# tingliu/glia

Measured on AMD Instinct MI355X. Metric: region_merges_per_sec, higher is better.
Workload: dtype u32 labels / f32 image / f64 statistics and features

## Files before the change

### glia_amd/csrc/api.cpp

```cpp
#include <algorithm>
#include <atomic>
#include <chrono>
#include <cmath>
#include <cstdio>
#include <cstdlib>
#include <cstring>
#include <limits>
#include <mutex>
#include <unordered_map>

#include "bc_features.hpp"
#include "forest.hpp"
#include "rmap_order.hpp"
#include "hmt_internal.hpp"

namespace glia {

static thread_local std::string g_err;
void set_error(const std::string& msg) { g_err = msg; }

static const char* const kOptionKeys[] = {"GLIA_HMT_PB_WINDOW", "GLIA_HMT_PB_BATCH", "GLIA_HMT_WINCAP", "GLIA_HMT_REBASE", "GLIA_HMT_HORIZON",
                                          "GLIA_HMT_FORCE_TREE", "GLIA_HMT_HELPERS", "GLIA_HMT_TRACE", "GLIA_HMT_LIBM", "GLIA_HMT_BC_NOCOMMON",
                                          "GLIA_HMT_BC_GENERIC", "GLIA_HMT_DEBUG", "GLIA_HMT_MAXITERS", "GLIA_HMT_MINCAP"};
static std::mutex g_opt_mu;
// ... 717 lines not shown
  }
  if (type != 1 && type != 2 && type != 3) {
    set_error("Error: unsupported boundary stats type...");
    return GLIA_HMT_ERR_ARG;
  }
  GLIA_HIP_TRY(hipSetDevice(c->device));
  *n_merges = 0;
  if (rag->arr.R == 0 || rag->arr.P == 0) return GLIA_HMT_OK;
  PbRequest req;
  if (type == 1 || type == 3) req.median_of = &rag->vol;
  req.size_weight = type == 3;
  MergeResult res;
  const int rc = greedy_mean(rag->arr, c->stream, req, &res);
  if (rc) return rc;
  rag->ms_table = res.ms_table; rag->ms_loop = res.ms_loop; rag->n_scored = res.n_scored;
  return order_to_keys(rag, res, "merge_order_pb", rag->only_contour, capacity, h_order, h_sal, n_merges);
}

static int upload_forest(const HostForest& hf, glia_hmt_forest* f, int slot, hipStream_t stream) {
  std::vector<PackedNode> nodes;
  std::vector<int> roots;
  int rc = pack_forest(hf, &nodes, &roots);
  if (rc) return rc;
  PackedNode* d_nodes = nullptr;
  int* d_roots = nullptr;
  GLIA_HIP_TRY(hipMalloc(&d_nodes, sizeof(PackedNode) * nodes.size()));
  f->allocs.push_back(d_nodes);
  GLIA_HIP_TRY(hipMalloc(&d_roots, sizeof(int) * roots.size()));
  f->allocs.push_back(d_roots);
  GLIA_HIP_TRY(hipMemcpyAsync(d_nodes, nodes.data(), sizeof(PackedNode) * nodes.size(), hipMemcpyHostToDevice, stream));
// ... 156 lines not shown
    set_error("pre_merge: invalid argument");
    return GLIA_HMT_ERR_ARG;
  }
  if (rag->only_contour) { set_error("pre_merge: the region map must hold region points (only_contour = 0)"); return GLIA_HMT_ERR_ARG; }
  GLIA_HIP_TRY(hipSetDevice(c->device));
  *n_merges = 0;
  if (rag->arr.R == 0 || rag->arr.P == 0) return GLIA_HMT_OK;
  PbRequest req;
  req.cond_n = n_thresholds;
  req.cond_sizes[0] = size_thresholds[0]; req.cond_sizes[1] = n_thresholds > 1 ? size_thresholds[1] : 0;
  req.cond_rpb = rpb_threshold;
  MergeResult res;
  const int rc = greedy_mean(rag->arr, c->stream, req, &res);
  if (rc) return rc;
  rag->ms_table = res.ms_table; rag->ms_loop = res.ms_loop; rag->n_scored = res.n_scored;
  return order_to_keys(rag, res, "pre_merge", false, capacity, h_order, h_sal, n_merges);
}

int glia_hmt_bc_feat(glia_hmt_ctx* c, glia_hmt_rag* rag, const uint32_t* h_order, int64_t n_merges, double* h_feats) {
  return glia_hmt_bc_feat_saliency(c, rag, h_order, n_merges, nullptr, 1.0, 1.0, h_feats);
}

int glia_hmt_bc_feat_dim(const glia_hmt_rag* rag, int with_saliency) {
  BcCfg cfg;
  if (!rag || !make_bc_cfg(rag, &cfg)) return -1;
  return cfg.fdim + median_extra_cols(rag, cfg) + ((with_saliency && !cfg.use_simple) ? 5 : 0);
}

int glia_hmt_bc_feat_saliency(glia_hmt_ctx* c, glia_hmt_rag* rag, const uint32_t* h_order, int64_t n_merges,
                              const double* h_saliencies, double init_saliency, double saliency_bias, double* h_feats) {
// ... 298 lines not shown
  if (!r || !out) return GLIA_HMT_ERR_ARG;
  *out = r->bcl;
  return GLIA_HMT_OK;
}

int glia_hmt_last_merge_timing(const glia_hmt_rag* r, double* ms_table, double* ms_init, double* ms_loop,
                               int64_t* n_scored) {
  if (!r) return GLIA_HMT_ERR_ARG;
  if (ms_table) *ms_table = r->ms_table;
  if (ms_init) *ms_init = r->ms_init;
  if (ms_loop) *ms_loop = r->ms_loop;
  if (n_scored) *n_scored = r->n_scored;
  return GLIA_HMT_OK;
}

}
```

### glia_amd/csrc/api_types.hpp

```cpp
#pragma once
#include "glibc_math.hpp"
#include "greedy_common.hpp"
#include "hmt_internal.hpp"

using namespace glia;

struct glia_hmt_ctx {
  int device = 0;
  hipStream_t stream = nullptr;
  bool own_stream = false;
  uint32_t rcap = 0, pcap = 0;
  uint32_t* rkeys = nullptr; uint32_t* rrec = nullptr;
  unsigned long long* pkeys = nullptr; uint32_t* prec = nullptr;
  uint32_t* flags = nullptr;
  hipEvent_t ev0 = nullptr, ev1 = nullptr;
  uint32_t hint_rcap = 0, hint_pcap = 0;
  double transform_ms = 0;
  int tz = kTZ;
  LibmSel libm = {kLibmDevice, kLibmDevice, kLibmDevice};
};

struct glia_hmt_rag {
  glia_hmt_ctx* ctx = nullptr;
  int dim = 3;
  int64_t dims[3] = {1, 1, 1};
  bool only_contour = false;
  int bins = 0, nthr = 0;
  RagArrays arr;
  double pass_ms = 0, alg_bytes = 0;
  double ms_table = 0, ms_init = 0, ms_loop = 0;
  glia_hmt_bc_label_timing bcl;
  int64_t n_scored = 0;
  glia_hmt_feat_config cfg;
  bool has_cfg = false;
  VolumeRef vol;
  VolumeRef slab;
  uint32_t* d_folded = nullptr;
  int map_region[GLIA_HMT_MAX_IMAGES] = {0}, map_rlabel[GLIA_HMT_MAX_IMAGES] = {0}, map_boundary[GLIA_HMT_MAX_IMAGES] = {0};
};
```

### glia_amd/csrc/greedy.hip

```cpp
#include <atomic>
#include <cstring>
#include <vector>
#include <limits>
#include <rocprim/device/device_scan.hpp>
#include <rocprim/device/device_radix_sort.hpp>
#include <rocprim/device/device_segmented_radix_sort.hpp>

#include "greedy_batch.hpp"

namespace glia {

__global__ void pq_build_level_kernel(PqTree t, int l) {
  const int lane = threadIdx.x & 63;
  uint32_t j = (blockIdx.x * blockDim.x + threadIdx.x) >> 6;
  if (j < t.lv[l].size) (void)pq_recompute_node(t, l, j, lane, true);
}

int pq_setup(DeviceBuffers& buf, PqTree& t, hipStream_t stream) {
  t.nlevels = 0;
  uint32_t n = t.nleaves;
  while (true) {
    n = (n + kFan - 1) / kFan;
    if (t.nlevels >= kMaxLevels) { set_error("greedy: edge table too large"); return GLIA_HMT_ERR_ARG; }
    PqLevel& L = t.lv[t.nlevels++];
// ... 22 lines not shown
namespace {

__global__ void win_range_kernel(const double* sal, uint32_t E0, unsigned long long* mm) {
  unsigned long long lo = ~0ull, hi = 0ull;
  for (uint32_t i = blockIdx.x * blockDim.x + threadIdx.x; i < E0; i += gridDim.x * blockDim.x) {
    const unsigned long long b = f64_ord(sal[i]);
    lo = b < lo ? b : lo; hi = b > hi ? b : hi;
  }
  atomicMin(&mm[0], lo); atomicMax(&mm[1], hi);
}
__global__ void win_params_kernel(const unsigned long long* mm, uint32_t B, double* range) {
  const double smin = f64_unord(mm[0]), smax = f64_unord(mm[1]);
  range[0] = smin;
  range[1] = smax > smin ? (double)B / (smax - smin) : 0.0;
}
__global__ void win_collect_kernel(const EdgeRec* er, uint32_t n_edges, const uint8_t* rdead, unsigned long long* kseq, uint32_t* vals, uint32_t* counter) {
  const uint32_t e = blockIdx.x * blockDim.x + threadIdx.x;
  if (e >= n_edges) return;
  const unsigned long long q = er[e].seq;
  if (q == 0) return;
  const uint2 uv = *reinterpret_cast<const uint2*>(&er[e].u);
  if (rdead[uv.x] | rdead[uv.y]) return;
  const uint32_t i = atomicAdd(counter, 1u);
  kseq[i] = q; vals[i] = e;
}
__global__ void win_salkey_kernel(const EdgeRec* er, const uint32_t* vals, uint32_t n, unsigned long long* ksal) {
  const uint32_t i = blockIdx.x * blockDim.x + threadIdx.x;
  if (i < n) ksal[i] = f64_ord(er[vals[i]].sal);
}
__global__ void win_baseline_fill_kernel(WinState st, uint32_t n, uint32_t* isort_w, unsigned long long* isort_seq) {
  const uint32_t i = blockIdx.x * blockDim.x + threadIdx.x;
  if (i >= n) return;
  const EdgeRec r = st.er[isort_w[i]];
  isort_seq[i] = r.seq;
  atomicAdd(&st.wcnt[win_cell(r.sal, st.wrange[0], st.wrange[1], st.wB)], 1u);
}
__global__ void win_segments_kernel(WinState st, const uint32_t* isort, uint32_t n, uint32_t* ige) {
  const uint32_t c = blockIdx.x * blockDim.x + threadIdx.x;
  if (c > st.wB) return;
// ... 128 lines not shown
  st.e_mean[e] = med;
  st.pq.leaf_sal[e] = st.size_weight ? -med * (double)min(st.rsz[st.e_u[e]], st.rsz[st.e_v[e]]) : -med;
  atomicAdd(&st.rbv[st.e_u[e]], (unsigned long long)n);
  atomicAdd(&st.rbv[st.e_v[e]], (unsigned long long)n);
}

__global__ void fill_leaves_dead(PqTree t, uint32_t from) {
  uint32_t i = from + blockIdx.x * blockDim.x + threadIdx.x;
  if (i < t.nleaves) { t.leaf_seq[i] = 0; t.leaf_sal[i] = -__builtin_inf(); }
}

}

struct WinBaseline {
  unsigned long long *kseq = nullptr, *kseq2 = nullptr, *ksal = nullptr, *ksal2 = nullptr, *iseq = nullptr;
  uint32_t *vals = nullptr, *vals2 = nullptr, *isort = nullptr, *ige = nullptr, *counter = nullptr;
  void* tmp = nullptr; size_t tmp_bytes = 0;
  uint32_t E0 = 0;
  double h_range[2] = {0.0, 0.0};
  long long prev_top_cell = -1;
  unsigned long long prev_ne = 0;
  double horizon_factor = 0.0;

  int init(DeviceBuffers& buf, WinState& ws, const double* leaf_sal, uint32_t n_initial, uint32_t B, uint32_t R, hipStream_t stream) {
    int rc;
    E0 = n_initial;
    unsigned long long* mm; double* range;
    if ((rc = buf.get(&ws.rdead, 2 * (size_t)R, true, stream))) return rc;
    if ((rc = buf.get(&ws.whead, B, false, stream))) return rc;
    if ((rc = buf.get(&ws.wcnt, B, true, stream))) return rc;
    if ((rc = buf.get(&isort, E0, false, stream))) return rc;
    if ((rc = buf.get(&iseq, E0, false, stream))) return rc;
    if ((rc = buf.get(&ige, (size_t)B + 1, false, stream))) return rc;
    if ((rc = buf.get(&mm, 2, false, stream))) return rc;
    if ((rc = buf.get(&range, 2, false, stream))) return rc;
    if ((rc = buf.get(&kseq, E0, false, stream))) return rc;
    if ((rc = buf.get(&kseq2, E0, false, stream))) return rc;
    if ((rc = buf.get(&ksal, E0, false, stream))) return rc;
    if ((rc = buf.get(&ksal2, E0, false, stream))) return rc;
    if ((rc = buf.get(&vals, E0, false, stream))) return rc;
    if ((rc = buf.get(&vals2, E0, false, stream))) return rc;
    if ((rc = buf.get(&counter, 1, true, stream))) return rc;
    GLIA_HIP_TRY(rocprim::radix_sort_pairs_desc(nullptr, tmp_bytes, kseq, kseq2, vals, vals2, (size_t)E0, 0, 64, stream));
    if ((rc = buf.get((char**)&tmp, tmp_bytes ? tmp_bytes : 16, false, stream))) return rc;
    ws.wrange = range; ws.isort = isort; ws.isort_seq = iseq; ws.ige = ige;
    const unsigned long long mm0[2] = {~0ull, 0ull};
    GLIA_HIP_TRY(hipMemcpyAsync(mm, mm0, sizeof(mm0), hipMemcpyHostToDevice, stream));
    hipLaunchKernelGGL(win_range_kernel, dim3(256), dim3(256), 0, stream, leaf_sal, E0, mm);
    hipLaunchKernelGGL(win_params_kernel, dim3(1), dim3(1), 0, stream, mm, B, range);
    GLIA_HIP_TRY(hipGetLastError());
    GLIA_HIP_TRY(hipMemcpyAsync(h_range, range, sizeof(h_range), hipMemcpyDeviceToHost, stream));
    GLIA_HIP_TRY(hipStreamSynchronize(stream));
    return GLIA_HMT_OK;
  }
  int rebaseline(WinState& ws, uint32_t n_edges, unsigned long long* ctrl, hipStream_t stream) {
    GLIA_HIP_TRY(hipMemsetAsync(counter, 0, sizeof(uint32_t), stream));
    hipLaunchKernelGGL(win_collect_kernel, dim3((n_edges + 255) / 256), dim3(256), 0, stream, ws.er, n_edges, ws.rdead, kseq, vals, counter);
    uint32_t n = 0;
    GLIA_HIP_TRY(hipMemcpyAsync(&n, counter, sizeof(uint32_t), hipMemcpyDeviceToHost, stream));
    GLIA_HIP_TRY(hipStreamSynchronize(stream));
    if (n > E0) { set_error("greedy: more live edges than initial edges (internal error)"); return GLIA_HMT_ERR_INTERNAL; }
    if (n) {
      size_t bytes = tmp_bytes;
      GLIA_HIP_TRY(rocprim::radix_sort_pairs_desc(tmp, bytes, kseq, kseq2, vals, vals2, (size_t)n, 0, 64, stream));
      hipLaunchKernelGGL(win_salkey_kernel, dim3((n + 255) / 256), dim3(256), 0, stream, ws.er, vals2, n, ksal);
      bytes = tmp_bytes;
      GLIA_HIP_TRY(rocprim::radix_sort_pairs_desc(tmp, bytes, ksal, ksal2, vals2, isort, (size_t)n, 0, 64, stream));
    }
    GLIA_HIP_TRY(hipMemsetAsync(ws.whead, 0xFF, sizeof(uint32_t) * ws.wB, stream));
    GLIA_HIP_TRY(hipMemsetAsync(ws.wcnt, 0, sizeof(uint32_t) * ws.wB, stream));
    if (n) hipLaunchKernelGGL(win_baseline_fill_kernel, dim3((n + 255) / 256), dim3(256), 0, stream, ws, n, isort, iseq);
    hipLaunchKernelGGL(win_segments_kernel, dim3((ws.wB + 1 + 255) / 256), dim3(256), 0, stream, ws, isort, n, ige);
    GLIA_HIP_TRY(hipGetLastError());
    ws.nsort = n;
    std::string renv;
    ws.rebase_after = option("GLIA_HMT_REBASE", &renv) ? strtoull(renv.c_str(), nullptr, 10) : std::max<unsigned long long>(800000ull, (unsigned long long)n / 2ull);
    ws.wch = 0;
    if (horizon_factor > 0.0 && n > 4096) {
      unsigned long long topkey = 0;
      GLIA_HIP_TRY(hipMemcpyAsync(&topkey, ksal2, sizeof(topkey), hipMemcpyDeviceToHost, stream));
      GLIA_HIP_TRY(hipStreamSynchronize(stream));
      const long long top_cell = (long long)win_cell(f64_unord(topkey), h_range[0], h_range[1], ws.wB);
      if (prev_top_cell >= 0 && n_edges > prev_ne) {
        const double d = (double)std::max<long long>(0, prev_top_cell - top_cell);
        const double delta = std::max(horizon_factor * d * (double)ws.rebase_after / (double)(n_edges - prev_ne), (double)ws.wB / 512.0);
        ws.wch = (double)top_cell > delta ? (uint32_t)((double)top_cell - delta) : 0u;
      }
      prev_top_cell = top_cell; prev_ne = n_edges;
    }
    ws.ne_base = n_edges;
    const double inf = std::numeric_limits<double>::infinity();
    ctrl[CTRL_CTHR] = (unsigned long long)(long long)(ws.wB - 1);
    memcpy(&ctrl[CTRL_TSAL], &inf, 8); ctrl[CTRL_TSEQ] = ~0ull; ctrl[CTRL_IPTR] = 0;
    return GLIA_HMT_OK;
  }
};
// ... 103 lines not shown
    ws.wB = B; ws.R0 = R;
    ws.wcap = kWinCap; ws.wbudget = kWinBudget;
    ws.force_tree = 0;
    if (option("GLIA_HMT_FORCE_TREE", &o_txt)) ws.force_tree = strtoull(o_txt.c_str(), nullptr, 10);
    if (option("GLIA_HMT_WINCAP", &o_txt)) {
      const uint32_t c = (uint32_t)strtoul(o_txt.c_str(), nullptr, 10);
      if (c >= 16 && c <= kWinCap) { ws.wcap = c; ws.wbudget = c / 2; }
    }
    ws.order = st.order; ws.sal_out = st.sal_out; ws.ctrl = st.ctrl; ws.rsz = st.rsz; ws.rsum = st.rsum;
    ws.mark0 = st.mark0; ws.mark1 = st.mark1; ws.adj_off = st.adj_off; ws.adj_len = st.adj_len;
    ws.pool_cap = st.pool_cap; ws.Ecap = st.Ecap;
    ws.cond_n = st.cond_n; ws.cond_t0 = st.cond_t0; ws.cond_t1 = st.cond_t1; ws.cond_rpb = st.cond_rpb;
    if ((rc = base.init(buf, ws, st.pq.leaf_sal, E0, B, R, stream))) return rc;
    if (req.cond_n <= 0 && !batch_off) base.horizon_factor = option("GLIA_HMT_HORIZON", &o_txt) ? atof(o_txt.c_str()) : 0.5;
    if ((rc = base.rebaseline(ws, E0, ctrl, stream))) return rc;
  } else if ((rc = pq_setup(buf, st.pq, stream))) return rc;
  GLIA_HIP_TRY(hipMemcpyAsync(st.ctrl, ctrl, sizeof(ctrl), hipMemcpyHostToDevice, stream));
  GLIA_HIP_TRY(hipEventRecord(ev.ev[1], stream));


  st.max_iters = window ? 1ull << 22 : 1ull << 16;
  const bool trace = option("GLIA_HMT_TRACE");
  if (option("GLIA_HMT_MAXITERS", &o_txt)) st.max_iters = std::max(1ull, strtoull(o_txt.c_str(), nullptr, 10));
  const auto kernel = [&]() { return !window ? "tree" : req.cond_n > 0 ? "window" : "batch"; };
  const auto unhandled = [&]() {
    set_error(std::string("greedy: the ") + kernel() + " kernel stopped with status " + std::to_string(ctrl[CTRL_STATUS]) + ", which its driver does not handle (internal error)");
    return GLIA_HMT_ERR_INTERNAL;
  };
  while (true) {
    if (window) {
      ws.max_iters = st.max_iters;
      if (req.cond_n > 0) hipLaunchKernelGGL(greedy_window_kernel<true>, dim3(1), dim3(kGreedyThreads), 0, stream, ws);
      else if (batch_off) hipLaunchKernelGGL(greedy_window_kernel<false>, dim3(1), dim3(kGreedyThreads), 0, stream, ws);
      else hipLaunchKernelGGL(greedy_batch_kernel, dim3(1), dim3(kGreedyThreads), 0, stream, ws);
    } else if (median_of) hipLaunchKernelGGL(greedy_pb_kernel<true>, dim3(1), dim3(kGreedyThreads), 0, stream, st);
    else hipLaunchKernelGGL(greedy_pb_kernel<false>, dim3(1), dim3(kGreedyThreads), 0, stream, st);
    GLIA_HIP_TRY(hipGetLastError());
    GLIA_HIP_TRY(hipMemcpyAsync(ctrl, st.ctrl, sizeof(ctrl), hipMemcpyDeviceToHost, stream));
    GLIA_HIP_TRY(hipStreamSynchronize(stream));
    if (trace) fprintf(stderr, "[trace] merge loop launch ended: status %llu, merges %llu of %u regions, edges %llu, list entries %llu\n", ctrl[CTRL_STATUS], ctrl[CTRL_MERGES], R, ctrl[CTRL_EDGES], ctrl[CTRL_ENTRIES]);
    if (ctrl[CTRL_STATUS] == ST_DONE) break;
    switch (ctrl[CTRL_STATUS]) {
      case ST_RUN:
        if (!window) continue;
        break;
      case ST_REBASE:
        if (!window) return unhandled();
        break;
      case ST_BAD_SALIENCY: set_error("Error: invalid boundary saliency..."); return GLIA_HMT_ERR_SALIENCY;
      case ST_INTERNAL: {
        char msg[256];
        snprintf(msg, sizeof(msg), "greedy: window queue overflow or more merges than regions (internal error: merges %llu of %u regions, %llu edges of %u initial, "
// ... 27 lines not shown
        break;
      }
      case ST_NEED_EDGES: {
        if (st.Ecap >= kMaxEdgeSlots) { set_error("greedy: more than 2^32 edge slots needed"); return GLIA_HMT_ERR_ARG; }
        const uint32_t ocap = st.Ecap, ncap = (uint32_t)std::min<unsigned long long>(kMaxEdgeSlots, (unsigned long long)ocap * 2ull);
        if ((rc = edges.grow(buf, ocap, ncap, stream))) return rc;
        st.Ecap = ncap; st.pq.nleaves = ncap; ws.Ecap = ncap;
        hipLaunchKernelGGL(fill_leaves_dead, dim3((ncap - ocap + 255) / 256), dim3(256), 0, stream, st.pq, ocap);
        if (!window && (rc = pq_setup(buf, st.pq, stream))) return rc;
        break;
      }
      default: return unhandled();
    }
    if (window) {
      if ((rc = base.rebaseline(ws, (uint32_t)ctrl[CTRL_EDGES], ctrl, stream))) return rc;
      GLIA_HIP_TRY(hipMemcpyAsync(st.ctrl + CTRL_CTHR, ctrl + CTRL_CTHR, 4 * sizeof(unsigned long long), hipMemcpyHostToDevice, stream));
    }
    unsigned long long zero = ST_RUN;
    GLIA_HIP_TRY(hipMemcpyAsync(st.ctrl + CTRL_STATUS, &zero, sizeof(zero), hipMemcpyHostToDevice, stream));
  }
  GLIA_HIP_TRY(hipEventRecord(ev.ev[2], stream));
  GLIA_HIP_TRY(hipEventSynchronize(ev.ev[2]));
  out->ms_table = ev.ms(0, 1); out->ms_loop = ev.ms(1, 2);
  out->n_scored = (int64_t)ctrl[CTRL_EDGES];
  return copy_merges(out, (int64_t)ctrl[CTRL_MERGES], st.order, st.sal_out);
}


static std::atomic<unsigned long long> g_internal_errors{0};
unsigned long long internal_errors() { return g_internal_errors.load(); }
void count_internal_error() { g_internal_errors.fetch_add(1); }
bool merge_order_is_consistent(const uint32_t* o, int64_t n, uint32_t R, int64_t* first_bad) {
  std::vector<uint8_t> gone(2 * (size_t)R + 1, 0);
  for (int64_t k = 0; k < n; ++k) {
    const uint32_t a = o[3 * k], b = o[3 * k + 1], c = o[3 * k + 2];
    if (k >= (int64_t)R || c != R + (uint32_t)k || a >= c || b >= c || a == b || gone[a] || gone[b]) { if (first_bad) *first_bad = k; return false; }
    gone[a] = gone[b] = 1;
  }
  return true;
// ... 17 lines not shown
```

### glia_amd/csrc/greedy_batch.hpp

```cpp
#pragma once
#include "greedy_window.hpp"

namespace glia {
namespace {

constexpr uint32_t kBatchKill = 32;
constexpr int kMemP = 3;
constexpr uint32_t kMemMax = 192;
struct BatchShared {
  alignas(16) Key part1[kNW];
  alignas(16) Key part2[kNW];
  uint32_t nkill, kovf; alignas(16) uint32_t kill[kBatchKill];
  uint32_t byrank[kNW];
  uint32_t bitmap[kNW][64];
  uint32_t m_newcount[kNW], m_total[kNW], m_ok[kNW];
  double m_maxsal[kNW];
  uint32_t bad;
};

template <int CTRL, int ROW_MASK = 0xf>
__device__ __forceinline__ void top2_ord_step(unsigned long long& a1, unsigned long long& a2) {
  const unsigned long long b1 = dpp64<CTRL, ROW_MASK, ROW_MASK != 0xf>(a1), b2 = dpp64<CTRL, ROW_MASK, ROW_MASK != 0xf>(a2);
  const bool g = b1 > a1;
  const unsigned long long hi = g ? b1 : a1, lo = g ? a1 : b1, m2 = b2 > a2 ? b2 : a2;
  a1 = hi; a2 = lo > m2 ? lo : m2;
}
__device__ __forceinline__ void wave_top2_ord(unsigned long long& a1, unsigned long long& a2) {
  top2_ord_step<0xB1>(a1, a2);
  top2_ord_step<0x4E>(a1, a2);
  top2_ord_step<0x124>(a1, a2);
  top2_ord_step<0x128>(a1, a2);
  top2_ord_step<0x142, 0xa>(a1, a2);
// ... 188 lines not shown
  lds_barrier();
  WIDE_T(5);
  if (tid == 0) { s.nitems = 0; s.newcount = 0; }
  *newcount_out = newcount;
  return total;
}

__global__ __launch_bounds__(kGreedyThreads) void greedy_batch_kernel(WinState st) {
  __shared__ WinShared w;
  __shared__ WinWork s;
  __shared__ BatchShared b;
  const int tid = threadIdx.x, lane = tid & 63, wave = tid >> 6;
  unsigned long long k = st.ctrl[CTRL_MERGES], ne = st.ctrl[CTRL_EDGES], pool_used = st.ctrl[CTRL_ENTRIES];
  uint32_t status = ST_RUN;
  win_enter(st, w, s, tid);
  if (tid == 0) { b.nkill = 0; b.kovf = 0; b.bad = 0; }
  b.bitmap[wave][lane] = 0;
  if (tid < kNW) { Key z; z.sal = -__builtin_inf(); z.seq = 0; z.arg = 0; b.part1[tid] = z; b.part2[tid] = z; }
  full_barrier();
  const double smin = st.wrange[0], scale = st.wrange[1];
  uint32_t pend_e = kNone, pend_old = kNone;
  constexpr uint32_t kTab = kMarkSlots / kNW;
  uint32_t* const tk = &s.mk[wave * kTab]; uint32_t* const t0 = &s.mv0[wave * kTab]; uint32_t* const t1 = &s.mv1[wave * kTab];
  static_assert(sizeof(s.stage) >= (size_t)kNW * kTab * 20, "per-wave staging");
  uint32_t* const sg_eid = reinterpret_cast<uint32_t*>(&s.stage[0]) + wave * kTab;
  uint32_t* const sg_n = reinterpret_cast<uint32_t*>(&s.stage[0]) + (kNW + wave) * kTab;
  uint32_t* const sg_pos = reinterpret_cast<uint32_t*>(&s.stage[0]) + (2 * kNW + wave) * kTab;
  double* const sg_mean = reinterpret_cast<double*>(reinterpret_cast<uint32_t*>(&s.stage[0]) + 3 * kNW * kTab) + wave * kTab;
#ifdef GLIA_HMT_PROFILE
  unsigned long long bph[8] = {0, 0, 0, 0, 0, 0, 0, 0}, blast = __builtin_readcyclecounter(), brounds = 0, bmembers = 0, bvalid = 0, bwide = 0, bcut_sal = 0, bcut_dep = 0;
  unsigned long long bw_n[4] = {0, 0, 0, 0}, bw_cyc[4] = {0, 0, 0, 0}, bw_ent[4] = {0, 0, 0, 0}, bw_new[4] = {0, 0, 0, 0};
// ... 46 lines not shown
    if (top_total > kMemMax) {
      if (ne + top_total > st.Ecap) { status = ST_NEED_EDGES; break; }
      if (pool_used + top_total > st.pool_cap) { status = ST_NEED_POOL; break; }
      uint32_t newcount = 0;
#ifdef GLIA_HMT_PROFILE
      const unsigned long long tw0 = __builtin_readcyclecounter();
#endif
      const uint32_t tt = batch_contract_wide(st, w, s, b, tid, top.arg, top.sal, k, ne, pool_used, smin, scale, &newcount);
      if (b.bad) { status = ST_BAD_SALIENCY; break; }
      k += 1; ne += newcount; pool_used += tt;
#ifdef GLIA_HMT_PROFILE
      bwide += 1;
      { const int cls = tt <= 512u ? 0 : tt <= kMarkMax ? 1 : tt <= 8192u ? 2 : 3; bw_n[cls] += 1; bw_cyc[cls] += __builtin_readcyclecounter() - tw0; bw_ent[cls] += tt; bw_new[cls] += newcount; }
#endif
      batch_scan(st, w, b, tid, kScanWide);
      if (w.spill_ord) { if (pend_e != kNone) { st.er[pend_e].next = pend_old; pend_e = kNone; } win_evict(st, w, tid); batch_scan(st, w, b, tid, kScanOther); }
      BPH(4);
      continue;
    }
    const bool narrow = member && total <= kMemMax;
    b.bitmap[wave][lane] = 0;
    FatEntry fe[kMemP];
    bool act[kMemP], side1[kMemP];
    uint32_t h[kMemP];
#pragma unroll
    for (int p = 0; p < kMemP; ++p) {
      const uint32_t i = (uint32_t)lane + 64u * (uint32_t)p;
      const bool inlist = narrow && i < total;
      side1[p] = i >= len0;
      fe[p].eid = kNone; fe[p].rs = 0; fe[p].n = 0; fe[p].pos = 0; fe[p].off = 0; fe[p].len = 0; fe[p].mean = 0.0;
      if (inlist) fe[p] = st.fpool[side1[p] ? off1 + (i - len0) : off0 + i];
// ... 73 lines not shown
      V = (uint32_t)__builtin_ctz(~okbits);
#ifdef GLIA_HMT_PROFILE
      if (V < M) { const uint32_t cutsal = (uint32_t)(__ballot(lane < kNW && j == V && !(kj.sal > pm)) & 0xFFull); if (cutsal) bcut_sal += 1; else bcut_dep += 1; }
#endif
      my_ne = (uint32_t)__builtin_amdgcn_readlane((int)pre_n, wave); my_pool = (uint32_t)__builtin_amdgcn_readlane((int)pre_t, wave);
      const uint32_t last = V - 1u;
      ne_off = (uint32_t)__shfl((int)(pre_n + nj), (int)last); pool_off = (uint32_t)__shfl((int)(pre_t + tj), (int)last);
    }
    const uint32_t sum_tot = pool_off;
    if (ne + sum_tot > st.Ecap) { status = ST_NEED_EDGES; break; }
    if (pool_used + sum_tot > st.pool_cap) { status = ST_NEED_POOL; break; }
    bool popped = false;
    if (wn_round + ne_off > st.wcap && wn_round > st.wcap / 2u) {
      if ((uint32_t)wave < V && lane == 0) w.seq[slot] = 0;
      popped = true;
      lds_barrier();
      win_compact(w, tid, st.wcap);
    }
    const WinTau tau = {w.cthr, w.tsal, w.tseq, smin, scale};
    BPH(2);
    if ((uint32_t)wave < V) {
      const unsigned long long kk = k + (unsigned long long)wave;
      const uint32_t r2 = st.R0 + (uint32_t)kk;
      const uint32_t r2off = (uint32_t)pool_used + my_pool;
      if (lane == 0) {
        if (!popped) w.seq[slot] = 0;
        st.order[3 * kk + 0] = r0; st.order[3 * kk + 1] = r1; st.order[3 * kk + 2] = r2;
        st.sal_out[kk] = me.sal;
        st.er[e].seq = 0;
        st.rdead[r0] = 1; st.rdead[r1] = 1;
// ... 10 lines not shown
        const unsigned long long seq = update_seq(kk, rs, r0, h0);
        const double sal = -first[p];
        store_new_edge(st, newE, rs, r2, posRs, idx[p], first[p], second[p], sal, seq, offRs, lenRs, r2off, newcount);
        win_queue_edge<true>(st, w, tau, newE, sal, seq, rs, r2, make_uint2(offRs, lenRs), make_uint2(r2off, newcount), pend_e, pend_old);
        win_retire_edge<true, false, kBatchKill>(st, tau, fe[p].eid, -fe[p].mean, &b.nkill, b.kill, &b.kovf);
        if (both[p]) win_retire_edge<true, false, kBatchKill>(st, tau, p_eid[p], -p_mean[p], &b.nkill, b.kill, &b.kovf);
      }
    }
    lds_barrier();
    BPH(3);
#ifdef GLIA_HMT_PROFILE
    brounds += 1; bmembers += M; bvalid += V;
#endif
    k += V; ne += ne_off; pool_used += pool_off;
    batch_scan(st, w, b, tid, kScanNarrow);
    if (w.spill_ord) { if (pend_e != kNone) { st.er[pend_e].next = pend_old; pend_e = kNone; } win_evict(st, w, tid); batch_scan(st, w, b, tid, kScanOther); }
    BPH(4);
  }
#ifdef GLIA_HMT_PROFILE
  if (tid == 0) printf("[batch profile] merges %llu: select %llu  compute %llu  validate %llu  commit %llu  scan %llu  loop-top %llu  reload %llu (cycles); rounds %llu candidates %llu committed %llu (cut by saliency %llu, by adjacency %llu) wide %llu\n",
                       k, bph[0], bph[1], bph[2], bph[3], bph[4], bph[5], bph[6], brounds, bmembers, bvalid, bcut_sal, bcut_dep, bwide);
  if (tid == 0) printf("[batch profile] scan phases (cumulative cycles, wave 0): loads %llu  compare %llu  top2 %llu  top2 with a tied best %llu  barrier %llu  calls %llu  tied second %llu  tied best %llu\n",
                       g_scanprof[0], g_scanprof[1], g_scanprof[2], g_scanprof[3], g_scanprof[4], g_scanprof[7], g_scanprof[5], g_scanprof[6]);
  if (tid == 0) printf("[batch profile] scan fill (cumulative; n <= 512, <= 1024, more): after reload/evict %llu %llu %llu  after narrow round %llu %llu %llu  after wide %llu %llu %llu\n",
                       g_scanfill[0][0], g_scanfill[0][1], g_scanfill[0][2], g_scanfill[1][0], g_scanfill[1][1], g_scanfill[1][2], g_scanfill[2][0], g_scanfill[2][1], g_scanfill[2][2]);
  if (tid == 0) printf("[batch profile] loop top (this launch): narrow rounds %llu cycles %llu  wide pops %llu cycles %llu\n", bsel_n[0], bsel[0], bsel_n[1], bsel[1]);
  if (tid == 0) printf("[batch profile] wide phases (cumulative cycles): entry-barrier %llu  lists+table %llu  compact %llu  main loop (wave 0) %llu  loop barrier %llu  tail %llu\n",
                       g_wideprof[0], g_wideprof[1], g_wideprof[2], g_wideprof[3], g_wideprof[4], g_wideprof[5]);
  if (tid == 0) printf("[batch profile] wide by entries (<=512, <=1408, <=8192, more): n %llu %llu %llu %llu  cycles %llu %llu %llu %llu  entries %llu %llu %llu %llu  new edges %llu %llu %llu %llu\n",
                       bw_n[0], bw_n[1], bw_n[2], bw_n[3], bw_cyc[0], bw_cyc[1], bw_cyc[2], bw_cyc[3], bw_ent[0], bw_ent[1], bw_ent[2], bw_ent[3], bw_new[0], bw_new[1], bw_new[2], bw_new[3]);
#endif
  if (pend_e != kNone) st.er[pend_e].next = pend_old;
  full_barrier();
  win_leave(st, w, tid, k, ne, pool_used, status);
}

}
}
```

### glia_amd/csrc/greedy_tree.hpp

```cpp
#pragma once
#include "greedy_common.hpp"

namespace glia {

struct GreedyState {
  uint32_t R0;
  uint32_t* adj_off;
  uint32_t* adj_len;
  uint2* pool;
  unsigned long long pool_cap;
  uint32_t Ecap;
  uint32_t *e_u, *e_v, *e_posu, *e_posv;
  double* e_mean;
  int* e_n;
  float* vals;
  unsigned long long vals_cap;
  unsigned long long* e_off;
  unsigned long long* rbv;
  int size_weight;
  PqTree pq;
  int cond_n; unsigned long long cond_t0, cond_t1; double cond_rpb;
  unsigned long long* rsz;
  double* rsum;
  uint32_t *mark0, *mark1;
  uint32_t* order;
  double* sal_out;
  unsigned long long* ctrl;
  unsigned long long max_iters;
};
enum { CTRL_MERGES = 0, CTRL_EDGES = 1, CTRL_ENTRIES = 2,
       CTRL_STATUS = 3, CTRL_VALUES = 4,
       CTRL_CTHR = 5, CTRL_TSAL = 6, CTRL_TSEQ = 7, CTRL_IPTR = 8,
       CTRL_WERR = 9, CTRL_WFILL = 10, CTRL_WORDS = 11 };

namespace {

__device__ __forceinline__ bool mean_link(bool h0, double m0, int n0, bool h1, double m1, int n1, double* first, int* second) {
  double f = 0.0;
  int sc = 0;
  if (h0) { f += m0 * n0; sc += n0; }
  if (h1) { f += m1 * n1; sc += n1; }
  f = sdivide(f, (double)sc, 0.0);
  *first = f; *second = sc;
  return f == -1.0;
}
__device__ __forceinline__ unsigned long long update_seq(unsigned long long k, uint32_t rs, uint32_t r0, bool h0) {
  const uint32_t cat = rs < r0 ? 0u : (h0 ? 1u : 2u);
  return ((k + 1ull) << 32) | ((unsigned long long)cat << 30) | rs;
// ... 358 lines not shown
```

### glia_amd/csrc/hmt_internal.hpp

```cpp
#pragma once
#include <hip/hip_runtime.h>
#include <stdint.h>
#include <string>
#include <vector>

#include "../../include/glia_hmt.h"

namespace glia {

void set_error(const std::string& msg);
bool option(const char* key, std::string* value = nullptr);
unsigned long long internal_errors();
void count_internal_error();
bool merge_order_is_consistent(const uint32_t* dense_order, int64_t n, uint32_t R, int64_t* first_bad);
int finish_merge_order(int rc, const uint32_t* dense_order, int64_t n, uint32_t R, hipStream_t stream);
#define GLIA_HIP_TRY(expr)                                                                       \
  do {                                                                                           \
    hipError_t _e = (expr);                                                                      \
    if (_e != hipSuccess) {                                                                      \
      ::glia::set_error(std::string(#expr) + ": " + hipGetErrorString(_e));                      \
      return GLIA_HMT_ERR_HIP;                                                                   \
    }                                                                                            \
  } while (0)

// ... 82 lines not shown
};
int median_feature_stats(const MedianFeatIn& in, hipStream_t stream, std::vector<double>* reg, std::vector<double>* bnd, std::vector<unsigned long long>* area);
struct TruthCount { uint32_t leaf, truth; unsigned long long count; };
int truth_overlap(const VolumeRef& vol, const uint32_t* d_rlabel, uint32_t R, const uint32_t* d_truth, hipStream_t stream,
                  std::vector<TruthCount>* out, float* ms);
struct NodeTruthStats { std::vector<unsigned long long> n, size, Q; std::vector<long double> E; };
void node_truth_stats(const std::vector<TruthCount>& cnt, uint32_t R, const uint32_t* forced, int64_t M, NodeTruthStats* out, int64_t* moves,
                      int64_t* node_pairs);
int bc_label_rules(const std::vector<NodeTruthStats>& st, uint32_t R, const uint32_t* forced, int64_t M, const glia_hmt_bc_label_opts& o,
                   int32_t* labels);
struct MergeResult {
  std::vector<uint32_t> order;
  std::vector<double> sal, rows;
  int64_t n = 0, n_scored = 0;
  double ms_table = 0.0, ms_init = 0.0, ms_loop = 0.0;
};
struct PbRequest {
  int cond_n = 0;
  long long cond_sizes[2] = {0, 0};
  double cond_rpb = 0.0;
  const VolumeRef* median_of = nullptr;
  bool size_weight = false;
};
int greedy_mean(const RagArrays& rag, hipStream_t stream, const PbRequest& req, MergeResult* out);
struct BcCfg;
struct DeviceClassifier;
struct BcRequest {
  const uint32_t* forced = nullptr;
  int64_t n_forced = 0;
  bool rows = false;
// ... 43 lines not shown
```

### glia_amd/hmt.py

```python
import ctypes as C
import os

import numpy as np

_HERE = os.path.dirname(os.path.abspath(__file__))
_SO = os.environ.get("GLIA_HMT_LIB", os.path.join(_HERE, "libglia_hmt.so"))

MAX_IMAGES, MAX_BINS, MAX_THRESH = 8, 16, 4


class HmtError(RuntimeError):
    def __init__(self, code, msg):
        super().__init__("glia_hmt error %d: %s" % (code, msg))
        self.code = code


class Image(C.Structure):
    _fields_ = [("d_image", C.c_void_p), ("bins", C.c_int), ("lo", C.c_double), ("hi", C.c_double)]


class FeatConfig(C.Structure):
    _fields_ = [
        ("n_region", C.c_int), ("region", Image * MAX_IMAGES),
        ("n_rlabel", C.c_int), ("rlabel", Image * MAX_IMAGES),
# ... 611 lines not shown

    def boundary_confidence(self, trees):
        import torch
        nt = len(trees)
        keep = [[np.ascontiguousarray(t[0], np.uint32), np.ascontiguousarray(t[1], np.int32), np.ascontiguousarray(t[2], np.int32),
                 np.ascontiguousarray(t[4], np.float64)] for t in trees]
        nn = (C.c_int64 * nt)(*[len(k[0]) for k in keep])
        arr = lambda j: (C.c_void_p * nt)(*[k[j].ctypes.data for k in keep])
        out = torch.empty(self.shape, dtype=torch.float32, device=torch.device("cuda", self.ctx.device))
        _check(lib().glia_hmt_boundary_confidence(self.ctx.h, self.h, C.c_int(nt), nn, arr(0), arr(1), arr(2), arr(3), C.c_void_p(out.data_ptr())))
        return out

    def last_merge_timing(self):
        a, b, c, n = C.c_double(), C.c_double(), C.c_double(), C.c_int64()
        _check(lib().glia_hmt_last_merge_timing(self.h, C.byref(a), C.byref(b), C.byref(c), C.byref(n)))
        return dict(ms_table=a.value, ms_init=b.value, ms_loop=c.value, n_edges_scored=n.value)
```

### include/glia_hmt.h

```cpp
#ifndef GLIA_HMT_H
#define GLIA_HMT_H

#include <stdint.h>

#ifdef __cplusplus
extern "C" {
#endif

#define GLIA_HMT_OK 0
#define GLIA_HMT_ERR_ARG (-1)
#define GLIA_HMT_ERR_HIP (-2)
#define GLIA_HMT_ERR_UNSUPPORTED (-3)
#define GLIA_HMT_ERR_CAPACITY (-4)
#define GLIA_HMT_ERR_SALIENCY (-5)
#define GLIA_HMT_ERR_IO (-6)
#define GLIA_HMT_ERR_INTERNAL (-7)

#define GLIA_HMT_MAX_IMAGES 8
#define GLIA_HMT_MAX_BINS 16
#define GLIA_HMT_MAX_THRESH 4

typedef struct glia_hmt_ctx glia_hmt_ctx;
typedef struct glia_hmt_rag glia_hmt_rag;
typedef struct glia_hmt_forest glia_hmt_forest;
// ... 162 lines not shown

int glia_hmt_relabel_image(glia_hmt_ctx* ctx, uint32_t* d_labels, int64_t n_voxels, int64_t min_size, uint32_t* n_labels);

double glia_hmt_last_transform_ms(const glia_hmt_ctx* ctx);

int64_t glia_hmt_gen_tree(const uint32_t* h_order, int64_t n_merges, uint32_t* node_label, int32_t* parent,
                          int32_t* child0, int32_t* child1, int64_t capacity);

int glia_hmt_score_initial_edges(glia_hmt_ctx* ctx, glia_hmt_rag* rag, const glia_hmt_forest* forest,
                                 int64_t* n_edges, double* ms);
int glia_hmt_score_initial_edges_shard(glia_hmt_ctx* ctx, glia_hmt_rag* rag, const glia_hmt_forest* forest, int shard,
                                       int n_shards, double* h_scores, int64_t capacity, int64_t* n_records);

int glia_hmt_last_merge_timing(const glia_hmt_rag* rag, double* ms_table, double* ms_init, double* ms_loop,
                               int64_t* n_edges_scored);

int glia_hmt_watershed(glia_hmt_ctx* ctx, int dim, const int64_t dims[3], const float* d_image, double level, uint32_t* d_labels,
                       uint32_t* n_labels, int* sweeps);

int glia_hmt_synth(glia_hmt_ctx* ctx, int dim, const int64_t dims[3], int S, int G, uint64_t seed,
                   int variant, uint32_t* d_labels, float* d_pb);

#ifdef __cplusplus
}
#endif
#endif
```

Before: 310,800.

## Rebuild window baseline incrementally from last sorted set plus new edges

The baseline collection now scans only the edges kept at the previous baseline plus the edge records created since, instead of every edge record. It uses wave-aggregated atomics to reserve output slots and computes the top saliency key in the same pass, which removes a separate device-to-host copy and stream sync. It also adds loop counters (launches, baselines, compactions, evictions) exposed through a new API call. The cost is more complex collection logic, a cap guard on writes, and a few extra LDS counters in the merge kernel.

```diff
diff --git a/glia_amd/csrc/api.cpp b/glia_amd/csrc/api.cpp
--- a/glia_amd/csrc/api.cpp
+++ b/glia_amd/csrc/api.cpp
@@ -755,6 +755,7 @@
   const int rc = greedy_mean(rag->arr, c->stream, req, &res);
   if (rc) return rc;
   rag->ms_table = res.ms_table; rag->ms_loop = res.ms_loop; rag->n_scored = res.n_scored;
+  rag->loop_counts[0] = res.launches; rag->loop_counts[1] = res.baselines; rag->loop_counts[2] = res.compactions; rag->loop_counts[3] = res.evictions;
   return order_to_keys(rag, res, "merge_order_pb", rag->only_contour, capacity, h_order, h_sal, n_merges);
 }
 
@@ -941,6 +942,7 @@
   const int rc = greedy_mean(rag->arr, c->stream, req, &res);
   if (rc) return rc;
   rag->ms_table = res.ms_table; rag->ms_loop = res.ms_loop; rag->n_scored = res.n_scored;
+  rag->loop_counts[0] = res.launches; rag->loop_counts[1] = res.baselines; rag->loop_counts[2] = res.compactions; rag->loop_counts[3] = res.evictions;
   return order_to_keys(rag, res, "pre_merge", false, capacity, h_order, h_sal, n_merges);
 }
 
@@ -1269,4 +1271,13 @@
   return GLIA_HMT_OK;
 }
 
-}
+int glia_hmt_last_merge_counts(const glia_hmt_rag* r, int64_t* launches, int64_t* baselines, int64_t* compactions, int64_t* evictions) {
+  if (!r) return GLIA_HMT_ERR_ARG;
+  if (launches) *launches = r->loop_counts[0];
+  if (baselines) *baselines = r->loop_counts[1];
+  if (compactions) *compactions = r->loop_counts[2];
+  if (evictions) *evictions = r->loop_counts[3];
+  return GLIA_HMT_OK;
+}
+
+}
diff --git a/glia_amd/csrc/api_types.hpp b/glia_amd/csrc/api_types.hpp
--- a/glia_amd/csrc/api_types.hpp
+++ b/glia_amd/csrc/api_types.hpp
@@ -31,6 +31,7 @@
   double ms_table = 0, ms_init = 0, ms_loop = 0;
   glia_hmt_bc_label_timing bcl;
   int64_t n_scored = 0;
+  int64_t loop_counts[4] = {0, 0, 0, 0};
   glia_hmt_feat_config cfg;
   bool has_cfg = false;
   VolumeRef vol;
diff --git a/glia_amd/csrc/greedy.hip b/glia_amd/csrc/greedy.hip
--- a/glia_amd/csrc/greedy.hip
+++ b/glia_amd/csrc/greedy.hip
@@ -60,15 +60,32 @@
   range[0] = smin;
   range[1] = smax > smin ? (double)B / (smax - smin) : 0.0;
 }
-__global__ void win_collect_kernel(const EdgeRec* er, uint32_t n_edges, const uint8_t* rdead, unsigned long long* kseq, uint32_t* vals, uint32_t* counter) {
-  const uint32_t e = blockIdx.x * blockDim.x + threadIdx.x;
-  if (e >= n_edges) return;
-  const unsigned long long q = er[e].seq;
-  if (q == 0) return;
-  const uint2 uv = *reinterpret_cast<const uint2*>(&er[e].u);
-  if (rdead[uv.x] | rdead[uv.y]) return;
-  const uint32_t i = atomicAdd(counter, 1u);
-  kseq[i] = q; vals[i] = e;
+__global__ void win_collect_kernel(const EdgeRec* er, const uint32_t* prev, uint32_t nprev, uint32_t e_from, uint32_t e_to, const uint8_t* rdead,
+                                   uint32_t cap, unsigned long long* kseq, uint32_t* vals, unsigned long long* stat) {
+  const unsigned long long i = (unsigned long long)blockIdx.x * blockDim.x + threadIdx.x;
+  const int lane = threadIdx.x & 63;
+  bool keep = i < (unsigned long long)nprev + (e_to - e_from);
+  uint32_t e = 0;
+  unsigned long long q = 0, o = 0;
+  if (keep) {
+    e = i < nprev ? prev[i] : e_from + (uint32_t)(i - nprev);
+    q = er[e].seq;
+    keep = q != 0;
+  }
+  if (keep) {
+    const uint2 uv = *reinterpret_cast<const uint2*>(&er[e].u);
+    keep = !(rdead[uv.x] | rdead[uv.y]);
+  }
+  if (keep) o = f64_ord(er[e].sal);
+  const unsigned long long m = __ballot(keep);
+  if (m == 0ull) return;
+  const unsigned long long top = wave_max_u64(o);
+  const int leader = (int)__builtin_ctzll(m);
+  unsigned long long base = 0;
+  if (lane == leader) { base = atomicAdd(&stat[0], (unsigned long long)__popcll(m)); atomicMax(&stat[1], top); }
+  base = lane_u64(base, leader);
+  const unsigned long long at = base + (unsigned long long)__popcll(m & ((1ull << lane) - 1ull));
+  if (keep && at < cap) { kseq[at] = q; vals[at] = e; }
 }
 __global__ void win_salkey_kernel(const EdgeRec* er, const uint32_t* vals, uint32_t n, unsigned long long* ksal) {
   const uint32_t i = blockIdx.x * blockDim.x + threadIdx.x;
@@ -227,7 +244,8 @@
 
 struct WinBaseline {
   unsigned long long *kseq = nullptr, *kseq2 = nullptr, *ksal = nullptr, *ksal2 = nullptr, *iseq = nullptr;
-  uint32_t *vals = nullptr, *vals2 = nullptr, *isort = nullptr, *ige = nullptr, *counter = nullptr;
+  uint32_t *vals = nullptr, *vals2 = nullptr, *isort = nullptr, *ige = nullptr;
+  unsigned long long* stat = nullptr;
   void* tmp = nullptr; size_t tmp_bytes = 0;
   uint32_t E0 = 0;
   double h_range[2] = {0.0, 0.0};
@@ -253,7 +271,7 @@
     if ((rc = buf.get(&ksal2, E0, false, stream))) return rc;
     if ((rc = buf.get(&vals, E0, false, stream))) return rc;
     if ((rc = buf.get(&vals2, E0, false, stream))) return rc;
-    if ((rc = buf.get(&counter, 1, true, stream))) return rc;
+    if ((rc = buf.get(&stat, 4, true, stream))) return rc;
     GLIA_HIP_TRY(rocprim::radix_sort_pairs_desc(nullptr, tmp_bytes, kseq, kseq2, vals, vals2, (size_t)E0, 0, 64, stream));
     if ((rc = buf.get((char**)&tmp, tmp_bytes ? tmp_bytes : 16, false, stream))) return rc;
     ws.wrange = range; ws.isort = isort; ws.isort_seq = iseq; ws.ige = ige;
@@ -267,11 +285,23 @@
     return GLIA_HMT_OK;
   }
   int rebaseline(WinState& ws, uint32_t n_edges, unsigned long long* ctrl, hipStream_t stream) {
-    GLIA_HIP_TRY(hipMemsetAsync(counter, 0, sizeof(uint32_t), stream));
-    hipLaunchKernelGGL(win_collect_kernel, dim3((n_edges + 255) / 256), dim3(256), 0, stream, ws.er, n_edges, ws.rdead, kseq, vals, counter);
-    uint32_t n = 0;
-    GLIA_HIP_TRY(hipMemcpyAsync(&n, counter, sizeof(uint32_t), hipMemcpyDeviceToHost, stream));
+    GLIA_HIP_TRY(hipMemsetAsync(stat, 0, 4 * sizeof(unsigned long long), stream));
+    const uint32_t nprev = ws.nsort, e_from = (uint32_t)ws.ne_base;
+    if (e_from > n_edges) { set_error("greedy: fewer edge records than at the last baseline (internal error)"); return GLIA_HMT_ERR_INTERNAL; }
+    const unsigned long long nscan = (unsigned long long)nprev + (n_edges - e_from);
+    if (nscan) hipLaunchKernelGGL(win_collect_kernel, dim3((unsigned)((nscan + 255) / 256)), dim3(256), 0, stream, ws.er, isort, nprev, e_from, n_edges, ws.rdead, E0, kseq, vals, stat);
+    unsigned long long h_stat[4] = {0, 0, 0, 0};
+#ifdef GLIA_HMT_PROFILE
+    if (n_edges) hipLaunchKernelGGL(win_collect_kernel, dim3((n_edges + 255) / 256), dim3(256), 0, stream, ws.er, isort, 0u, 0u, n_edges, ws.rdead, E0, kseq2, vals2, stat + 2);
+#endif
+    GLIA_HIP_TRY(hipMemcpyAsync(h_stat, stat, sizeof(h_stat), hipMemcpyDeviceToHost, stream));
     GLIA_HIP_TRY(hipStreamSynchronize(stream));
+#ifdef GLIA_HMT_PROFILE
+    fprintf(stderr, "[baseline profile] incremental collection: %llu items from %llu records; full collection: %llu items from %u records\n", h_stat[0], nscan, h_stat[2], n_edges);
+    if (h_stat[0] != h_stat[2] || h_stat[1] != h_stat[3]) { set_error("greedy: the incremental baseline collection differs from the full one (internal error)"); return GLIA_HMT_ERR_INTERNAL; }
+#endif
+    if (option("GLIA_HMT_TRACE")) fprintf(stderr, "[trace] baseline: %llu items of %llu records read (%u of the last baseline, %u created since; %u exist)\n", h_stat[0], nscan, nprev, n_edges - e_from, n_edges);
+    const uint32_t n = (uint32_t)std::min<unsigned long long>(h_stat[0], (unsigned long long)E0 + 1ull);
     if (n > E0) { set_error("greedy: more live edges than initial edges (internal error)"); return GLIA_HMT_ERR_INTERNAL; }
     if (n) {
       size_t bytes = tmp_bytes;
@@ -290,9 +320,7 @@
     ws.rebase_after = option("GLIA_HMT_REBASE", &renv) ? strtoull(renv.c_str(), nullptr, 10) : std::max<unsigned long long>(800000ull, (unsigned long long)n / 2ull);
     ws.wch = 0;
     if (horizon_factor > 0.0 && n > 4096) {
-      unsigned long long topkey = 0;
-      GLIA_HIP_TRY(hipMemcpyAsync(&topkey, ksal2, sizeof(topkey), hipMemcpyDeviceToHost, stream));
-      GLIA_HIP_TRY(hipStreamSynchronize(stream));
+      const unsigned long long topkey = h_stat[1];
       const long long top_cell = (long long)win_cell(f64_unord(topkey), h_range[0], h_range[1], ws.wB);
       if (prev_top_cell >= 0 && n_edges > prev_ne) {
         const double d = (double)std::max<long long>(0, prev_top_cell - top_cell);
@@ -426,6 +454,7 @@
     if ((rc = base.init(buf, ws, st.pq.leaf_sal, E0, B, R, stream))) return rc;
     if (req.cond_n <= 0 && !batch_off) base.horizon_factor = option("GLIA_HMT_HORIZON", &o_txt) ? atof(o_txt.c_str()) : 0.5;
     if ((rc = base.rebaseline(ws, E0, ctrl, stream))) return rc;
+    out->baselines = 1;
   } else if ((rc = pq_setup(buf, st.pq, stream))) return rc;
   GLIA_HIP_TRY(hipMemcpyAsync(st.ctrl, ctrl, sizeof(ctrl), hipMemcpyHostToDevice, stream));
   GLIA_HIP_TRY(hipEventRecord(ev.ev[1], stream));
@@ -448,6 +477,7 @@
     } else if (median_of) hipLaunchKernelGGL(greedy_pb_kernel<true>, dim3(1), dim3(kGreedyThreads), 0, stream, st);
     else hipLaunchKernelGGL(greedy_pb_kernel<false>, dim3(1), dim3(kGreedyThreads), 0, stream, st);
     GLIA_HIP_TRY(hipGetLastError());
+    out->launches += 1;
     GLIA_HIP_TRY(hipMemcpyAsync(ctrl, st.ctrl, sizeof(ctrl), hipMemcpyDeviceToHost, stream));
     GLIA_HIP_TRY(hipStreamSynchronize(stream));
     if (trace) fprintf(stderr, "[trace] merge loop launch ended: status %llu, merges %llu of %u regions, edges %llu, list entries %llu\n", ctrl[CTRL_STATUS], ctrl[CTRL_MERGES], R, ctrl[CTRL_EDGES], ctrl[CTRL_ENTRIES]);
@@ -505,6 +535,7 @@
     }
     if (window) {
       if ((rc = base.rebaseline(ws, (uint32_t)ctrl[CTRL_EDGES], ctrl, stream))) return rc;
+      out->baselines += 1;
       GLIA_HIP_TRY(hipMemcpyAsync(st.ctrl + CTRL_CTHR, ctrl + CTRL_CTHR, 4 * sizeof(unsigned long long), hipMemcpyHostToDevice, stream));
     }
     unsigned long long zero = ST_RUN;
@@ -514,6 +545,7 @@
   GLIA_HIP_TRY(hipEventSynchronize(ev.ev[2]));
   out->ms_table = ev.ms(0, 1); out->ms_loop = ev.ms(1, 2);
   out->n_scored = (int64_t)ctrl[CTRL_EDGES];
+  out->compactions = (int64_t)ctrl[CTRL_NPOPPED]; out->evictions = (int64_t)ctrl[CTRL_NEVICT];
   return copy_merges(out, (int64_t)ctrl[CTRL_MERGES], st.order, st.sal_out);
 }
 
diff --git a/glia_amd/csrc/greedy_batch.hpp b/glia_amd/csrc/greedy_batch.hpp
--- a/glia_amd/csrc/greedy_batch.hpp
+++ b/glia_amd/csrc/greedy_batch.hpp
@@ -16,6 +16,7 @@
   uint32_t m_newcount[kNW], m_total[kNW], m_ok[kNW];
   double m_maxsal[kNW];
   uint32_t bad;
+  uint32_t n_popped, n_evict;
 };
 
 template <int CTRL, int ROW_MASK = 0xf>
@@ -234,7 +235,7 @@
   unsigned long long k = st.ctrl[CTRL_MERGES], ne = st.ctrl[CTRL_EDGES], pool_used = st.ctrl[CTRL_ENTRIES];
   uint32_t status = ST_RUN;
   win_enter(st, w, s, tid);
-  if (tid == 0) { b.nkill = 0; b.kovf = 0; b.bad = 0; }
+  if (tid == 0) { b.nkill = 0; b.kovf = 0; b.bad = 0; b.n_popped = 0; b.n_evict = 0; }
   b.bitmap[wave][lane] = 0;
   if (tid < kNW) { Key z; z.sal = -__builtin_inf(); z.seq = 0; z.arg = 0; b.part1[tid] = z; b.part2[tid] = z; }
   full_barrier();
@@ -311,7 +312,7 @@
       { const int cls = tt <= 512u ? 0 : tt <= kMarkMax ? 1 : tt <= 8192u ? 2 : 3; bw_n[cls] += 1; bw_cyc[cls] += __builtin_readcyclecounter() - tw0; bw_ent[cls] += tt; bw_new[cls] += newcount; }
 #endif
       batch_scan(st, w, b, tid, kScanWide);
-      if (w.spill_ord) { if (pend_e != kNone) { st.er[pend_e].next = pend_old; pend_e = kNone; } win_evict(st, w, tid); batch_scan(st, w, b, tid, kScanOther); }
+      if (w.spill_ord) { if (pend_e != kNone) { st.er[pend_e].next = pend_old; pend_e = kNone; } if (tid == 0) b.n_evict += 1; win_evict(st, w, tid); batch_scan(st, w, b, tid, kScanOther); }
       BPH(4);
       continue;
     }
@@ -415,6 +416,7 @@
     if (wn_round + ne_off > st.wcap && wn_round > st.wcap / 2u) {
       if ((uint32_t)wave < V && lane == 0) w.seq[slot] = 0;
       popped = true;
+      if (tid == 0) b.n_popped += 1;
       lds_barrier();
       win_compact(w, tid, st.wcap);
     }
@@ -455,7 +457,7 @@
 #endif
     k += V; ne += ne_off; pool_used += pool_off;
     batch_scan(st, w, b, tid, kScanNarrow);
-    if (w.spill_ord) { if (pend_e != kNone) { st.er[pend_e].next = pend_old; pend_e = kNone; } win_evict(st, w, tid); batch_scan(st, w, b, tid, kScanOther); }
+    if (w.spill_ord) { if (pend_e != kNone) { st.er[pend_e].next = pend_old; pend_e = kNone; } if (tid == 0) b.n_evict += 1; win_evict(st, w, tid); batch_scan(st, w, b, tid, kScanOther); }
     BPH(4);
   }
 #ifdef GLIA_HMT_PROFILE
@@ -473,6 +475,7 @@
 #endif
   if (pend_e != kNone) st.er[pend_e].next = pend_old;
   full_barrier();
+  if (tid == 0) { st.ctrl[CTRL_NPOPPED] += b.n_popped; st.ctrl[CTRL_NEVICT] += b.n_evict; }
   win_leave(st, w, tid, k, ne, pool_used, status);
 }
 
diff --git a/glia_amd/csrc/greedy_tree.hpp b/glia_amd/csrc/greedy_tree.hpp
--- a/glia_amd/csrc/greedy_tree.hpp
+++ b/glia_amd/csrc/greedy_tree.hpp
@@ -31,7 +31,8 @@
 enum { CTRL_MERGES = 0, CTRL_EDGES = 1, CTRL_ENTRIES = 2,
        CTRL_STATUS = 3, CTRL_VALUES = 4,
        CTRL_CTHR = 5, CTRL_TSAL = 6, CTRL_TSEQ = 7, CTRL_IPTR = 8,
-       CTRL_WERR = 9, CTRL_WFILL = 10, CTRL_WORDS = 11 };
+       CTRL_WERR = 9, CTRL_WFILL = 10,
+       CTRL_NPOPPED = 11, CTRL_NEVICT = 12, CTRL_WORDS = 13 };
 
 namespace {
 
diff --git a/glia_amd/csrc/hmt_internal.hpp b/glia_amd/csrc/hmt_internal.hpp
--- a/glia_amd/csrc/hmt_internal.hpp
+++ b/glia_amd/csrc/hmt_internal.hpp
@@ -120,6 +120,7 @@
   std::vector<double> sal, rows;
   int64_t n = 0, n_scored = 0;
   double ms_table = 0.0, ms_init = 0.0, ms_loop = 0.0;
+  int64_t launches = 0, baselines = 0, compactions = 0, evictions = 0;
 };
 struct PbRequest {
   int cond_n = 0;
diff --git a/glia_amd/hmt.py b/glia_amd/hmt.py
--- a/glia_amd/hmt.py
+++ b/glia_amd/hmt.py
@@ -649,4 +649,7 @@
     def last_merge_timing(self):
         a, b, c, n = C.c_double(), C.c_double(), C.c_double(), C.c_int64()
         _check(lib().glia_hmt_last_merge_timing(self.h, C.byref(a), C.byref(b), C.byref(c), C.byref(n)))
-        return dict(ms_table=a.value, ms_init=b.value, ms_loop=c.value, n_edges_scored=n.value)
+        k = [C.c_int64() for _ in range(4)]
+        _check(lib().glia_hmt_last_merge_counts(self.h, *[C.byref(x) for x in k]))
+        return dict(ms_table=a.value, ms_init=b.value, ms_loop=c.value, n_edges_scored=n.value,
+                    launches=k[0].value, baselines=k[1].value, compactions=k[2].value, evictions=k[3].value)
diff --git a/include/glia_hmt.h b/include/glia_hmt.h
--- a/include/glia_hmt.h
+++ b/include/glia_hmt.h
@@ -200,6 +200,7 @@
 
 int glia_hmt_last_merge_timing(const glia_hmt_rag* rag, double* ms_table, double* ms_init, double* ms_loop,
                                int64_t* n_edges_scored);
+int glia_hmt_last_merge_counts(const glia_hmt_rag* rag, int64_t* launches, int64_t* baselines, int64_t* compactions, int64_t* evictions);
 
 int glia_hmt_watershed(glia_hmt_ctx* ctx, int dim, const int64_t dims[3], const float* d_image, double level, uint32_t* d_labels,
                        uint32_t* n_labels, int* sweeps);
```

Measured after the change: 313,200 (median of 6 runs). Within noise of the previous version (+0.8%).
